# ssilverman16/particle_col_image_segmentation

Hardware: AMD Instinct MI355X
Metric: Mpixels/sec segmented (5-ch 1024x1024 TIFF), ROI mask IoU=1.0 (higher is better)
Workload: dtype f32 planes / u8 class maps / int32 labels / f64 ROI sums; 1 GPU; BASELINE config 2: batch of 64 frames 1024x1024x5 float32 per GPU, full kernel chain, inputs resident in HBM; frames_per_gpu=64, height=1024, width=1024, planes=5, parallelism=frames x1, launch=one hipGraph replay per step, 4 in flight, tie_fallback_frames_last_step=0, reference_nan_frames_rank0=0

## Files before the change

particle_col_image_segmentation_amd/csrc/ccl.hip:

```cpp
#include <type_traits>

#include "column_pass.h"
#include "tile_ops.h"

namespace pcseg {

constexpr int SCAN_PIX = 1024;

struct KeyEqU8 {
    const uint8_t *p;
    int W;
    int64_t n;
    __device__ __forceinline__ int operator()(int b, int r, int c) const { return p[b * n + rowoff(r, W) + c]; }
};
struct KeyNzU8 {
    const uint8_t *p;
    int W;
    int64_t n;
    __device__ __forceinline__ int operator()(int b, int r, int c) const { return p[b * n + rowoff(r, W) + c] != 0; }
};
struct KeyZeroU8 {
    const uint8_t *p;
    int W;
    int64_t n;
// ... 376 lines not shown
    const size_t words = (size_t)B * ((H + 31) / 32) * W;
    DilateCclWs ws;
    ws.bits = cv.take<unsigned>(words);
    ws.dil = cv.take<unsigned>(words);
    return ws;
}
static unsigned *dilate_ccl_runs_carve(Carver &cv, int B, int H, int W) { return cv.take<unsigned>((size_t)B * ((H + 31) / 32) * W); }

struct FillHolesWs : CclWs {
    uint8_t *flag;
};
static FillHolesWs fill_holes_carve(Carver &cv, int B, int H, int W)
{
    FillHolesWs ws;
    static_cast<CclWs &>(ws) = ccl_carve(cv, B, H, W);
    ws.flag = cv.take<uint8_t>((size_t)B * H * W);
    return ws;
}

struct LocmaxWs : CclWs {
    size_t nwords;
    unsigned long long *cbits;
    uint8_t *bad;
    int *nonconst;
};
static LocmaxWs locmax_carve(Carver &cv, int B, int H, int W)
{
    const size_t total = (size_t)B * H * W;
    LocmaxWs ws;
    static_cast<CclWs &>(ws) = ccl_carve(cv, B, H, W);
    ws.nwords = (total + 63) / 64;
    ws.cbits = cv.take<unsigned long long>(ws.nwords + 1);
    ws.bad = cv.take<uint8_t>(total);
    ws.nonconst = cv.take<int>(B);
    return ws;
}

struct OverlapWs : CclWs {
    int *area, *ov;
};
static OverlapWs overlap_carve(Carver &cv, int B, int H, int W)
{
    OverlapWs ws;
    static_cast<CclWs &>(ws) = ccl_carve(cv, B, H, W);
    ws.area = cv.take<int>((size_t)B * H * W);
    ws.ov = cv.take<int>((size_t)B * H * W);
    return ws;
}

template <typename KeyFn, bool CONN8>
static int ccl_roots(KeyFn keyfn, int *parent, int B, int H, int W, hipStream_t s, bool tile_pass_done = false, int *corrupt = nullptr)
{
    if (corrupt) PCSEG_CHECK_HIP(hipMemsetAsync(corrupt, 0, sizeof(int) * (size_t)B, s));
    dim3 tgrid((W + CCL_TW - 1) / CCL_TW, (H + CCL_TH - 1) / CCL_TH, B);
    if (!tile_pass_done) {
        PCSEG_LAUNCH((ccl_tile_kernel<KeyFn, CONN8>), tgrid, dim3(256), 0, s, keyfn, parent, H, W);
        PCSEG_CHECK_LAUNCH();
    }
    if (tgrid.x > 1 || tgrid.y > 1) {
        const int64_t border_px = (int64_t)((H - 1) / CCL_TH) * W + (int64_t)(CONN8 ? 2 : 1) * ((W - 1) / CCL_TW) * H;
        dim3 bgrid((unsigned)((border_px + 255) / 256), B);
        PCSEG_LAUNCH((ccl_border_kernel<KeyFn, CONN8>), bgrid, dim3(256), 0, s, keyfn, parent, H, W, corrupt);
        PCSEG_CHECK_LAUNCH();
    }
    return PCSEG_OK;
}

template <typename Pred>
static int ccl_compact(int *parent, int *blockcount, int nblk, int *labels, int *counts, Pred pred, bool flatten,
                       int B, int H, int W, hipStream_t s, int *corrupt = nullptr)
{
    int64_t n = (int64_t)H * W;
    dim3 grid(nblk, B);
    PCSEG_LAUNCH((ccl_flatten_count_kernel<Pred>), grid, dim3(256), 0, s, parent, labels, blockcount, pred, n, nblk, false, corrupt);
    PCSEG_CHECK_LAUNCH();
    PCSEG_LAUNCH(ccl_scan_blocks_kernel, dim3(B), dim3(256), 0, s, blockcount, counts, nblk, (const int *)corrupt);
    PCSEG_CHECK_LAUNCH();
    if ((n & 3) == 0 && (((uintptr_t)parent | (uintptr_t)labels) & 15) == 0) {
        const dim3 qgrid((unsigned)((n + SCAN_PIX * RELABEL_Q - 1) / (SCAN_PIX * RELABEL_Q)), B);
        PCSEG_LAUNCH((ccl_relabel_quads_kernel<Pred>), qgrid, dim3(256), 0, s, (const int *)parent, labels, (const int *)blockcount, pred, n,
                     nblk, flatten, counts);
    } else {
        PCSEG_LAUNCH((ccl_relabel_kernel<Pred>), grid, dim3(256), 0, s, (const int *)parent, labels, (const int *)blockcount, pred, n, nblk,
                     flatten, counts);
    }
    PCSEG_CHECK_LAUNCH();
    return PCSEG_OK;
}

template <typename KeyFn, bool CONN8>
static int ccl_full(KeyFn keyfn, int32_t *labels, int32_t *counts, int B, int H, int W, void *workspace,
                    size_t workspace_bytes, hipStream_t s)
{
    Carver cv(workspace, workspace_bytes);
    CclWs ws = ccl_carve(cv, B, H, W);
    if (!cv.ok()) {
        set_error("ccl: workspace too small (%zu < %zu)", workspace_bytes, cv.off);
        return PCSEG_ERR_WORKSPACE;
    }
    int rc = ccl_roots<KeyFn, CONN8>(keyfn, ws.parent, B, H, W, s, false, ws.corrupt);
    if (rc) return rc;
    return ccl_compact(ws.parent, ws.blockcount, ws.nblk, labels, counts, PredAll(), true, B, H, W, s, ws.corrupt);
}

int ccl_plan(void *workspace, size_t workspace_bytes, int B, int H, int W, CclPlan *plan, const char *who)
{
    Carver cv(workspace, workspace_bytes);
    CclWs ws = ccl_carve(cv, B, H, W);
    if (!cv.ok()) {
        set_error("%s: workspace too small (%zu < %zu)", who, workspace_bytes, cv.off);
        return PCSEG_ERR_WORKSPACE;
    }
    plan->parent = ws.parent;
    plan->blockcount = ws.blockcount;
    plan->nblk = ws.nblk;
    plan->corrupt = ws.corrupt;
    return PCSEG_OK;
}

int ccl_equal_u8_finish(const uint8_t *in, const CclPlan &plan, bool tile_pass_done, int *labels, int *counts, int B, int H, int W,
                        hipStream_t s)
{
    const KeyEqU8 keyfn{in, W, (int64_t)H * W};
    PCSEG_CHECK_HIP(hipMemsetAsync(plan.corrupt, 0, sizeof(int) * (size_t)B, s));
    dim3 tgrid((W + CCL_TW - 1) / CCL_TW, (H + CCL_TH - 1) / CCL_TH, B);
    if (!tile_pass_done) {
        PCSEG_LAUNCH((ccl_tile_kernel<KeyEqU8, true>), tgrid, dim3(256), 0, s, keyfn, plan.parent, H, W);
        PCSEG_CHECK_LAUNCH();
    }
    if (tgrid.x > 1 || tgrid.y > 1) {
        const int64_t border_px = (int64_t)((H - 1) / CCL_TH) * W + (int64_t)2 * ((W - 1) / CCL_TW) * H;
        dim3 bgrid((unsigned)((border_px + 255) / 256), B);
        PCSEG_LAUNCH((ccl_border_kernel<KeyEqU8, true>), bgrid, dim3(256), 0, s, keyfn, plan.parent, H, W, plan.corrupt);
        PCSEG_CHECK_LAUNCH();
    }
    return ccl_compact(plan.parent, plan.blockcount, plan.nblk, labels, counts, PredAll(), true, B, H, W, s, plan.corrupt);
}

__global__ void __launch_bounds__(256) roots_to_parent_kernel(const int *__restrict__ roots, int *__restrict__ parent, int64_t total)
{
    int64_t i = (int64_t)blockIdx.x * blockDim.x + threadIdx.x;
    if (i < total) parent[i] = roots[i] - 1;
}

struct MaskSet {
    unsigned long long bits[4];
    int n;
};
template <bool VEC>
__global__ void __launch_bounds__(256) set_bits_kernel(const uint8_t *__restrict__ in, MaskSet masks, unsigned *__restrict__ bits,
                                                        int H, int W, int nch, int B)
{
    constexpr int COLS = VEC ? 4 : 1;
    const int c = (blockIdx.x * 256 + threadIdx.x) * COLS;
    const int ch = blockIdx.y, b = blockIdx.z;
    if (c >= W) return;
    const uint8_t *src = in + (int64_t)b * H * W + c;
    unsigned w[4][COLS];
#pragma unroll
    for (int m = 0; m < 4; ++m)
#pragma unroll
        for (int j = 0; j < COLS; ++j) w[m][j] = 0;
#pragma unroll 1
    for (int j0 = 0; j0 < 32; j0 += 8) {
        unsigned v8[8];
#pragma unroll
        for (int j = 0; j < 8; ++j) {
            const uint8_t *at = src + rowoff(min(ch * 32 + j0 + j, H - 1), W);
            v8[j] = VEC ? *reinterpret_cast<const unsigned *>(at) : (unsigned)*at;
        }
#pragma unroll
        for (int j = 0; j < 8; ++j) {
#pragma unroll
            for (int q = 0; q < COLS; ++q) {
                const unsigned a = (v8[j] >> (8 * q)) & 255u;
                const unsigned long long sel = a < 64 ? (1ull << a) : 0ull;
#pragma unroll
                for (int m = 0; m < 4; ++m)
                    if (m < masks.n && (masks.bits[m] & sel)) w[m][q] |= 1u << (j0 + j);
            }
        }
    }
    {
        const int rows = min(32, H - ch * 32);
        const unsigned valid = col_valid(rows);
#pragma unroll
        for (int m = 0; m < 4; ++m)
#pragma unroll
            for (int q = 0; q < COLS; ++q) w[m][q] &= valid;
    }
    const int64_t plane = (int64_t)B * nch * W;
#pragma unroll
    for (int m = 0; m < 4; ++m)
        if (m < masks.n) {
            unsigned *out = bits + m * plane + ((int64_t)b * nch + ch) * W + c;
            if constexpr (VEC) *reinterpret_cast<uint4 *>(out) = make_uint4(w[m][0], w[m][1], w[m][2], w[m][3]);
            else *out = w[m][0];
        }
}

__global__ void __launch_bounds__(256) dilate_bits_kernel(const unsigned *__restrict__ in, unsigned *__restrict__ out,
                                                           int radius, int H, int W, int nch)
{
    const int c = blockIdx.x * 256 + threadIdx.x;
    const int ch = blockIdx.y, b = blockIdx.z;
    if (c >= W) return;
    const unsigned *base = in + (int64_t)b * nch * W;
    unsigned acc = 0;
    for (int dy = 0; dy <= radius; ++dy) {
        int half = 0;
        while ((half + 1) * (half + 1) + dy * dy <= radius * radius) ++half;
        unsigned cur = 0, prev = 0, next = 0;
        for (int dx = -half; dx <= half; ++dx) {
            int cc = c + dx;
            if (cc < 0 || cc >= W) continue;
            cur |= base[rowoff(ch, W) + cc];
            if (dy > 0) {
                if (ch > 0) prev |= base[rowoff((ch - 1), W) + cc];
                if (ch + 1 < nch) next |= base[rowoff((ch + 1), W) + cc];
            }
        }
        if (dy == 0) acc |= cur;
        else {
            acc |= (cur << dy) | (prev >> (32 - dy));
            acc |= (cur >> dy) | (next << (32 - dy));
        }
    }
    const int rows = min(32, H - ch * 32);
    acc &= col_valid(rows);
    out[((int64_t)b * nch + ch) * W + c] = acc;
}

__global__ void __launch_bounds__(256) dilate_bits_disk2_kernel(const unsigned *__restrict__ in, unsigned *__restrict__ out, int H, int W,
                                                                 int nch)
{
    const int c = blockIdx.x * 256 + threadIdx.x;
    const int ch = blockIdx.y, b = blockIdx.z;
    if (c >= W) return;
    const unsigned *base = in + (int64_t)b * nch * W;
    const int chu = max(ch - 1, 0), chd = min(ch + 1, nch - 1);
    const unsigned *rc = base + rowoff(ch, W), *ru = base + rowoff(chu, W), *rd = base + rowoff(chd, W);
    const int c1l = max(c - 1, 0), c2l = max(c - 2, 0), c1r = min(c + 1, W - 1), c2r = min(c + 2, W - 1);
    const unsigned w0 = rc[c], w1l = rc[c1l], w1r = rc[c1r], w2l = rc[c2l], w2r = rc[c2r];
    unsigned u0 = ru[c], u1l = ru[c1l], u1r = ru[c1r], d0 = rd[c], d1l = rd[c1l], d1r = rd[c1r];
    if (ch == 0) u0 = u1l = u1r = 0;
    if (ch + 1 >= nch) d0 = d1l = d1r = 0;
    const unsigned cur1 = w0 | w1l | w1r, prev1 = u0 | u1l | u1r, next1 = d0 | d1l | d1r;
    unsigned acc = cur1 | w2l | w2r;
    acc |= (cur1 << 1) | (prev1 >> 31) | (cur1 >> 1) | (next1 << 31);
    acc |= (w0 << 2) | (u0 >> 30) | (w0 >> 2) | (d0 << 30);
    const int rows = min(32, H - ch * 32);
    acc &= col_valid(rows);
    out[((int64_t)b * nch + ch) * W + c] = acc;
}

constexpr int BR_TW = 64, BR_CH = 4, BR_ROWS = 32 * BR_CH;

__device__ __forceinline__ int bitrun_start(unsigned word, int p)
{
    const unsigned below = ~word & ((1u << p) - 1u);
    return below ? 32 - __clz(below) : 0;
}

template <typename Link>
__device__ __forceinline__ void bitrun_left_links(unsigned w, unsigned wl, Link &&link)
{
    unsigned rest = wl ? w : 0u;
    while (rest) {
        const int a = __ffs(rest) - 1;
        const unsigned from_a = w >> a;
        const int len = from_a == 0xFFFFFFFFu ? 32 : __ffs(~from_a) - 1;
        const int e = a + len - 1;
        rest = e >= 31 ? 0u : rest & ~((2u << e) - 1u);
        const int lo = max(a - 1, 0), hi = min(e + 1, 31);
        unsigned m = wl & (hi == 31 ? 0xFFFFFFFFu : ((2u << hi) - 1u)) & ~((1u << lo) - 1u);
        while (m) {
            const int p = __ffs(m) - 1;
            const int st = bitrun_start(wl, p);
            const unsigned from_p = wl >> p;
            const int run_len = from_p == 0xFFFFFFFFu ? 32 : __ffs(~from_p) - 1;
            const int en = p + run_len - 1;
            m = en >= 31 ? 0u : m & ~((2u << en) - 1u);
            link(a, st);
        }
    }
}

__global__ void __launch_bounds__(256) bitrun_tile_kernel(const unsigned *__restrict__ bits, int *__restrict__ parent, int H, int W,
                                                           int nch)
{
    __shared__ unsigned sw[BR_CH][BR_TW];
    __shared__ int lpar[BR_ROWS * BR_TW];
    const int col = threadIdx.x & (BR_TW - 1), q = threadIdx.x >> 6;
    const int c0 = blockIdx.x * BR_TW, ch0 = blockIdx.y * BR_CH, b = blockIdx.z;
    const int c = c0 + col, ch = ch0 + q;
    const unsigned w = (c < W && ch < nch) ? bits[((int64_t)b * nch + ch) * W + c] : 0u;
    sw[q][col] = w;
    for (unsigned heads = w & ~(w << 1); heads; heads &= heads - 1) {
        const int node = (q * 32 + (__ffs(heads) - 1)) * BR_TW + col;
        lpar[node] = node;
    }
    __syncthreads();
    if (w) {
        if (col > 0)
            bitrun_left_links(w, sw[q][col - 1], [&](int a, int st) {
                unite_lds(lpar, (q * 32 + a) * BR_TW + col, (q * 32 + st) * BR_TW + col - 1);
            });
        if ((w & 1u) && q > 0) {
            const int node = (q * 32) * BR_TW + col;
            const unsigned wu = sw[q - 1][col];
            if (wu >> 31) {
                unite_lds(lpar, node, ((q - 1) * 32 + bitrun_start(wu, 31)) * BR_TW + col);
            } else {
                if (col > 0 && (sw[q - 1][col - 1] >> 31))
                    unite_lds(lpar, node, ((q - 1) * 32 + bitrun_start(sw[q - 1][col - 1], 31)) * BR_TW + col - 1);
                if (col + 1 < BR_TW && (sw[q - 1][col + 1] >> 31))
                    unite_lds(lpar, node, ((q - 1) * 32 + bitrun_start(sw[q - 1][col + 1], 31)) * BR_TW + col + 1);
            }
        }
    }
    __syncthreads();
    int *par = parent + (int64_t)b * H * W;
    for (unsigned heads = w & ~(w << 1); heads; heads &= heads - 1) {
        const int node = (q * 32 + (__ffs(heads) - 1)) * BR_TW + col;
        const int root = find_lds(lpar, node);
        par[(ch0 * 32 + node / BR_TW) * W + c0 + node % BR_TW] = (ch0 * 32 + root / BR_TW) * W + c0 + root % BR_TW;
    }
}

__global__ void __launch_bounds__(256) bitrun_border_kernel(const unsigned *__restrict__ bits, int *__restrict__ parent, int H, int W,
                                                             int nch)
{
    const int c = blockIdx.x * 256 + threadIdx.x;
    const int ch = blockIdx.y, b = blockIdx.z;
    if (c >= W) return;
    const int col = c & (BR_TW - 1);
    const bool tile_left = col == 0 && c > 0, tile_top = (ch % BR_CH) == 0 && ch > 0;
    const bool edge_col = col == 0 || col == BR_TW - 1;
    if (!tile_left && !tile_top && !(edge_col && ch > 0)) return;
    const unsigned *wb = bits + (int64_t)b * nch * W;
    const int cl = c > 0 ? c - 1 : c, cr = c + 1 < W ? c + 1 : c, chu = ch > 0 ? ch - 1 : ch;
    const unsigned w = wb[rowoff(ch, W) + c], wl = wb[rowoff(ch, W) + cl];
    const unsigned wu = wb[rowoff(chu, W) + c], wul = wb[rowoff(chu, W) + cl], wur = wb[rowoff(chu, W) + cr];
    if (w == 0) return;
    int *par = parent + (int64_t)b * H * W;
    const int row0 = ch * 32;
    if (tile_left)
        bitrun_left_links(w, wl, [&](int a, int st) { unite_glb(par, (row0 + a) * W + c, (row0 + st) * W + c - 1); });
    if ((w & 1u) && ch > 0) {
        const int node = row0 * W + c;
        if (wu >> 31) {
            if (tile_top) unite_glb(par, node, (row0 - 32 + bitrun_start(wu, 31)) * W + c);
        } else {
            if (c > 0 && (tile_top || col == 0) && (wul >> 31)) unite_glb(par, node, (row0 - 32 + bitrun_start(wul, 31)) * W + c - 1);
            if (c + 1 < W && (tile_top || col == BR_TW - 1) && (wur >> 31))
                unite_glb(par, node, (row0 - 32 + bitrun_start(wur, 31)) * W + c + 1);
        }
    }
}

__global__ void __launch_bounds__(256) border_flag_kernel(const int *__restrict__ parent, uint8_t *__restrict__ flag, int H, int W)
{
    int t = blockIdx.x * blockDim.x + threadIdx.x;
    int r, c;
    if (t < W) { r = 0; c = t; }
    else if (t < 2 * W) { r = H - 1; c = t - W; }
    else if (t < 2 * W + H) { r = t - 2 * W; c = 0; }
    else if (t < 2 * W + 2 * H) { r = t - 2 * W - H; c = W - 1; }
    else return;
    int64_t fbase = (int64_t)blockIdx.y * H * W;
    int p = parent[fbase + rowoff(r, W) + c];
    if (p >= 0) flag[fbase + p] = 1;
}

__global__ void __launch_bounds__(256) fill_holes_out_kernel(const uint8_t *__restrict__ mask, const int *__restrict__ parent,
                                                              const uint8_t *__restrict__ flag, uint8_t *__restrict__ out, int64_t n)
{
    int64_t i = (int64_t)blockIdx.x * blockDim.x + threadIdx.x;
    if (i >= n) return;
    int64_t fbase = (int64_t)blockIdx.y * n;
    int p = parent[fbase + i];
    out[fbase + i] = (mask[fbase + i] != 0) || (p >= 0 && flag[fbase + p] == 0);
}

__global__ void __launch_bounds__(256) ccl_flatten_kernel(int *__restrict__ parent, int64_t n)
{
    int64_t i = (int64_t)blockIdx.x * blockDim.x + threadIdx.x;
    if (i >= n) return;
    int *par = parent + (int64_t)blockIdx.y * n;
    int p = par[i];
    if (p < 0 || !walk_ok((int)i, p)) return;
    const int x = walk_root(par, p);
    if (x != p) par[i] = x;
}

constexpr int LM_TW = CCL_TW, LM_TH = CCL_TH, LM_SW = LM_TW + 4, LM_SH = LM_TH + 4, LM_CW = LM_TW + 2, LM_CH = LM_TH + 2;

__global__ void __launch_bounds__(256) locmax_candidates_kernel(const int *__restrict__ img, unsigned long long *__restrict__ cbits,
                                                                 uint8_t *__restrict__ bad, int *__restrict__ nonconst,
                                                                 int *__restrict__ parent, int *__restrict__ markers, int H, int W)
{
    __shared__ int tile[LM_SH * LM_SW];
    __shared__ uint8_t cand[LM_CH * LM_CW];
    __shared__ int key[CCL_TILE];
    static_assert(LM_SH * LM_SW >= CCL_TILE, "the parents reuse the value tile");
    int *par = tile;
    const int OUTSIDE = (int)0x80000000;
    const TileIndex ti = xcd_tile_index();
    const int r0 = ti.y * LM_TH, c0 = ti.x * LM_TW;
    const int64_t fbase = (int64_t)ti.z * H * W;
    if ((W & 3) == 0 && c0 + LM_TW <= W && (((uintptr_t)img) & 15) == 0) {
        constexpr int QUADS = LM_SH * (LM_TW / 4), TRIPS = (QUADS + 255) / 256;
        int4 tq[TRIPS];
#pragma unroll
        for (int t = 0; t < TRIPS; ++t) {
            const int i = min((int)threadIdx.x + 256 * t, QUADS - 1);
            const int r = r0 + i / (LM_TW / 4) - 2;
            tq[t] = *reinterpret_cast<const int4 *>(img + fbase + rowoff(min(max(r, 0), H - 1), W) + c0 + 4 * (i % (LM_TW / 4)));
        }
        const int hl = min((int)threadIdx.x, LM_SH * 4 - 1);
        const int hr = r0 + (hl >> 2) - 2, hx = (hl & 3) < 2 ? (hl & 3) - 2 : LM_TW + (hl & 3) - 2, hc = c0 + hx;
        const int hv = img[fbase + rowoff(min(max(hr, 0), H - 1), W) + min(max(hc, 0), W - 1)];
#pragma unroll
        for (int t = 0; t < TRIPS; ++t) {
            const int i = (int)threadIdx.x + 256 * t;
            if (i < QUADS) {
                const int lr = i / (LM_TW / 4), r = r0 + lr - 2;
                const bool in = r >= 0 && r < H;
                int *dst = tile + lr * LM_SW + 2 + 4 * (i % (LM_TW / 4));
                dst[0] = in ? tq[t].x : OUTSIDE; dst[1] = in ? tq[t].y : OUTSIDE; dst[2] = in ? tq[t].z : OUTSIDE; dst[3] = in ? tq[t].w : OUTSIDE;
            }
        }
        if (threadIdx.x < LM_SH * 4) tile[(hl >> 2) * LM_SW + hx + 2] = (hr >= 0 && hr < H && hc >= 0 && hc < W) ? hv : OUTSIDE;
    } else {
        constexpr int TRIPS = (LM_SH * LM_SW + 255) / 256;
        int tv[TRIPS];
#pragma unroll
        for (int t = 0; t < TRIPS; ++t) {
            const int i = min((int)threadIdx.x + 256 * t, LM_SH * LM_SW - 1);
            const int r = r0 + i / LM_SW - 2, c = c0 + i % LM_SW - 2;
            tv[t] = img[fbase + rowoff(min(max(r, 0), H - 1), W) + min(max(c, 0), W - 1)];
        }
#pragma unroll
        for (int t = 0; t < TRIPS; ++t) {
            const int i = (int)threadIdx.x + 256 * t;
            const int r = r0 + i / LM_SW - 2, c = c0 + i % LM_SW - 2;
            if (i < LM_SH * LM_SW) tile[i] = (r >= 0 && r < H && c >= 0 && c < W) ? tv[t] : OUTSIDE;
        }
    }
    __syncthreads();
    const int first_value = img[fbase];
    bool any_differs = false;
    for (int t = threadIdx.x; t < LM_CH * LM_CW; t += 256) {
        const int lr = t / LM_CW, lc = t % LM_CW;
        const int r = r0 + lr - 1, c = c0 + lc - 1;
        const int i = (lr + 1) * LM_SW + lc + 1;
        const int v = tile[i];
        uint8_t state = 2;
        if (r >= 0 && r < H && c >= 0 && c < W) {
            const int *up = tile + i - LM_SW, *dn = tile + i + LM_SW;
            const int m = max(max(max(up[-1], up[0]), max(up[1], tile[i - 1])), max(max(tile[i + 1], dn[-1]), max(dn[0], dn[1])));
            state = m < v ? 1 : (m == v ? 3 : 0);
            any_differs = any_differs || v != first_value;
        }
        cand[t] = state;
    }
    __syncthreads();
    unsigned links = 0;
#pragma unroll
    for (int kk = 0; kk < LM_TH * LM_TW / 256; ++kk) {
        const int t = threadIdx.x + 256 * kk;
        const int lr = t / LM_TW, lc = t % LM_TW;
        const int r = r0 + lr, c = c0 + lc;
        int k = 0;
        if (r < H && c < W) {
            const int i = (lr + 2) * LM_SW + lc + 2, j = (lr + 1) * LM_CW + lc + 1;
            const int v = tile[i];
            const uint8_t st = cand[j];
            const bool is_cand = (st & 1) != 0;
            bool touches = false;
            if (st == 3) {
#pragma unroll
                for (int dr = -1; dr <= 1; ++dr)
#pragma unroll
                    for (int dc = -1; dc <= 1; ++dc) {
                        if (dr == 0 && dc == 0) continue;
                        const bool eq = tile[i + dr * LM_SW + dc] == v;
                        const uint8_t sn = cand[j + dr * LM_CW + dc];
                        touches = touches || (eq && sn == 0);
                        if ((dr < 0 || (dr == 0 && dc < 0)) && eq && (sn & 1) && lr + dr >= 0 && lc + dc >= 0 && lc + dc < LM_TW)
                            links |= 1u << (4 * kk + (dr == 0 ? 0 : dc + 2));
                    }
// ... 64 lines not shown
    uint8_t v = 0;
    if (cand_bit(cbits, fbase + i)) v = bad[fbase + parent[fbase + i]] == 0 && nonconst[blockIdx.y] != 0;
    is_max[fbase + i] = v;
}

__device__ __forceinline__ unsigned long long cand_word(const unsigned long long *cbits, int b, int64_t i0, int64_t n)
{
    if (i0 >= n) return 0ull;
    const int64_t g0 = (int64_t)b * n + i0;
    const int sh = (int)(g0 & 63);
    unsigned long long w = cbits[g0 >> 6] >> sh;
    if (sh) w |= cbits[(g0 >> 6) + 1] << (64 - sh);
    if (n - i0 < 64) w &= (1ull << (n - i0)) - 1ull;
    return w;
}

static_assert(SCAN_PIX == 1024, "sixteen 64-bit words per count block");
template <typename Pred>
__global__ void __launch_bounds__(256) locmax_count_kernel(const int *__restrict__ parent, int *__restrict__ labels,
                                                            int *__restrict__ blockcount, const unsigned long long *__restrict__ cbits,
                                                            Pred pred, int64_t n, int nblk)
{
    const int b = blockIdx.y;
    const int *par = parent + (int64_t)b * n;
    const int64_t word = (int64_t)blockIdx.x * 256 + threadIdx.x;
    const int64_t i0 = word * 64;
    unsigned long long roots = 0;
    for (unsigned long long m = cand_word(cbits, b, i0, n); m; m &= m - 1) {
        const int j = __ffsll((long long)m) - 1;
        const int64_t i = i0 + j;
        if (par[i] == (int)i && pred((int64_t)b * n + i)) roots |= 1ull << j;
    }
    const int cnt = __popcll(roots);
    int inc = cnt;
    for (int off = 1; off < 16; off <<= 1) {
        const int t = __shfl_up(inc, off, 16);
        if ((threadIdx.x & 15) >= off) inc += t;
    }
    int rank = inc - cnt;
    for (unsigned long long m = roots; m; m &= m - 1) labels[(int64_t)b * n + i0 + (__ffsll((long long)m) - 1)] = -(++rank);
    if ((threadIdx.x & 15) == 15 && word / 16 < nblk) blockcount[b * nblk + (int)(word / 16)] = inc;
}

template <typename Pred>
__global__ void __launch_bounds__(256) locmax_relabel_kernel(const int *__restrict__ parent, int *labels, const int *__restrict__ blockoff,
                                                              const unsigned long long *__restrict__ cbits, Pred pred, int64_t n, int nblk)
{
    const int b = blockIdx.y;
    const int *par = parent + (int64_t)b * n;
    int *lab = labels + (int64_t)b * n;
    const int64_t i0 = ((int64_t)blockIdx.x * 256 + threadIdx.x) * 64;
    for (unsigned long long m = cand_word(cbits, b, i0, n); m; m &= m - 1) {
        const int64_t i = i0 + (__ffsll((long long)m) - 1);
        const int p = par[i];
        int v = 0;
        if (pred((int64_t)b * n + p)) {
            v = __hip_atomic_load(lab + p, __ATOMIC_RELAXED, __HIP_MEMORY_SCOPE_WORKGROUP);
            if (v < 0) v = blockoff[b * nblk + p / SCAN_PIX] - v;
        }
        lab[i] = v;
    }
}

__global__ void __launch_bounds__(256) overlap_count_kernel(const int *__restrict__ parent, const uint8_t *__restrict__ other,
                                                             int *__restrict__ area, int *__restrict__ ov, int64_t n)
{
    int64_t i = (int64_t)blockIdx.x * blockDim.x + threadIdx.x;
    if (i >= n) return;
    int64_t fbase = (int64_t)blockIdx.y * n;
    int p = parent[fbase + i];
    if (p < 0) return;
    atomicAdd(&area[fbase + p], 1);
    if (other[fbase + i] == 1) atomicAdd(&ov[fbase + p], 1);
}

__global__ void __launch_bounds__(256) overlap_out_kernel(const uint8_t *__restrict__ dapi, const int *__restrict__ parent,
                                                           const int *__restrict__ area, const int *__restrict__ ov,
                                                           double threshold, uint8_t *__restrict__ out, int64_t n)
{
    int64_t i = (int64_t)blockIdx.x * blockDim.x + threadIdx.x;
    if (i >= n) return;
    int64_t fbase = (int64_t)blockIdx.y * n;
    int p = parent[fbase + i];
    uint8_t v = dapi[fbase + i];
    if (p >= 0) {
        double frac = (double)ov[fbase + p] / (double)area[fbase + p];
        if (frac > threshold) v = 2;
    }
    out[fbase + i] = v;
}

}

using namespace pcseg;

extern "C" {

size_t pcseg_ccl_workspace_bytes(int B, int H, int W)
{
    if (!check_shape(B, H, W)) return 0;
    Carver cv(nullptr, 0);
    ccl_carve(cv, B, H, W);
    return cv.off;
}

int pcseg_ccl8_equal_u8(const uint8_t *in, int32_t *labels, int32_t *counts, int B, int H, int W, void *workspace,
                        size_t workspace_bytes, pcseg_stream_t stream)
{
    PCSEG_REQUIRE(in && labels && counts && workspace && check_shape(B, H, W), "bad arguments");
    return ccl_full<KeyEqU8, true>(KeyEqU8{in, W, (int64_t)H * W}, labels, counts, B, H, W, workspace, workspace_bytes, (hipStream_t)stream);
}

int pcseg_ccl8_bool(const uint8_t *in, int32_t *labels, int32_t *counts, int B, int H, int W, void *workspace,
                    size_t workspace_bytes, pcseg_stream_t stream)
{
    PCSEG_REQUIRE(in && labels && counts && workspace && check_shape(B, H, W), "bad arguments");
    return ccl_full<KeyNzU8, true>(KeyNzU8{in, W, (int64_t)H * W}, labels, counts, B, H, W, workspace, workspace_bytes, (hipStream_t)stream);
}

int pcseg_ccl4_bool(const uint8_t *in, int32_t *labels, int32_t *counts, int B, int H, int W, void *workspace,
                    size_t workspace_bytes, pcseg_stream_t stream)
{
    PCSEG_REQUIRE(in && labels && counts && workspace && check_shape(B, H, W), "bad arguments");
    return ccl_full<KeyNzU8, false>(KeyNzU8{in, W, (int64_t)H * W}, labels, counts, B, H, W, workspace, workspace_bytes, (hipStream_t)stream);
}

size_t pcseg_dilate_ccl_workspace_bytes(int B, int H, int W)
{
    if (!check_shape(B, H, W)) return 0;
    Carver cv(nullptr, 0);
    dilate_ccl_carve(cv, B, H, W);
    return cv.off;
}

static int dilated_bit_planes(const uint8_t *in, const MaskSet &masks, int radius, unsigned *bits, unsigned *dil, int B, int H, int W,
                              hipStream_t s)
{
    const int nch = (H + 31) / 32;
    if ((W & 3) == 0 && ((uintptr_t)in & 3) == 0 && ((uintptr_t)bits & 15) == 0)
        PCSEG_LAUNCH(set_bits_kernel<true>, dim3((W / 4 + 255) / 256, nch, B), dim3(256), 0, s, in, masks, bits, H, W, nch, B);
    else
        PCSEG_LAUNCH(set_bits_kernel<false>, dim3((W + 255) / 256, nch, B), dim3(256), 0, s, in, masks, bits, H, W, nch, B);
    PCSEG_CHECK_LAUNCH();
    const dim3 g((W + 255) / 256, nch, B * masks.n);
    if (radius == 2) PCSEG_LAUNCH(dilate_bits_disk2_kernel, g, dim3(256), 0, s, (const unsigned *)bits, dil, H, W, nch);
    else PCSEG_LAUNCH(dilate_bits_kernel, g, dim3(256), 0, s, (const unsigned *)bits, dil, radius, H, W, nch);
    PCSEG_CHECK_LAUNCH();
    return PCSEG_OK;
}

static int bitrun_components(const unsigned *dil, int *run_parent, int B, int H, int W, hipStream_t s)
{
    const int nch = (H + 31) / 32;
    PCSEG_LAUNCH(bitrun_tile_kernel, dim3((W + BR_TW - 1) / BR_TW, (nch + BR_CH - 1) / BR_CH, B), dim3(256), 0, s, dil, run_parent, H,
                 W, nch);
    PCSEG_CHECK_LAUNCH();
    PCSEG_LAUNCH(bitrun_border_kernel, dim3((W + 255) / 256, nch, B), dim3(256), 0, s, dil, run_parent, H, W, nch);
    PCSEG_CHECK_LAUNCH();
    return PCSEG_OK;
}

static MaskSet mask_set(const uint64_t *value_bits, int n_masks)
{
    MaskSet masks;
    masks.n = n_masks;
    for (int m = 0; m < 4; ++m) masks.bits[m] = m < n_masks ? (unsigned long long)value_bits[m] : 0ull;
    return masks;
}

int pcseg_dilate_ccl_roots_u8(const uint8_t *in, uint64_t value_bits, int radius, int32_t *roots, int B, int H, int W,
                              void *workspace, size_t workspace_bytes, pcseg_stream_t stream)
{
    PCSEG_REQUIRE(in && roots && workspace && radius >= 0 && radius <= 15 && check_shape(B, H, W), "bad arguments (radius <= 15)");
    hipStream_t s = (hipStream_t)stream;
    Carver cv(workspace, workspace_bytes);
    const DilateCclWs ws = dilate_ccl_carve(cv, B, H, W);
    if (!cv.ok()) {
        set_error("dilate_ccl_roots: workspace too small (%zu < %zu)", workspace_bytes, cv.off);
        return PCSEG_ERR_WORKSPACE;
    }
    const int rc = dilated_bit_planes(in, mask_set(&value_bits, 1), radius, ws.bits, ws.dil, B, H, W, s);
    if (rc) return rc;
    return ccl_roots<KeyBits, true>(KeyBits{ws.dil, W, (H + 31) / 32}, roots, B, H, W, s);
}

size_t pcseg_dilate_ccl_runs_workspace_bytes(int B, int H, int W)
{
    if (!check_shape(B, H, W)) return 0;
    Carver cv(nullptr, 0);
    dilate_ccl_runs_carve(cv, B, H, W);
    return cv.off;
}

int pcseg_dilate_ccl_runs_multi_u8(const uint8_t *in, const uint64_t *value_bits, int n_masks, int radius, uint32_t *dilated_bits,
                                   int32_t *run_parent, int B, int H, int W, void *workspace, size_t workspace_bytes,
                                   pcseg_stream_t stream)
{
    PCSEG_REQUIRE(in && value_bits && dilated_bits && run_parent && workspace && n_masks >= 1 && n_masks <= 4 && radius >= 0 &&
                      radius <= 15 && check_shape(B, H, W) && check_shape(B * n_masks, H, W),
                  "bad arguments (1..4 masks, radius <= 15)");
    hipStream_t s = (hipStream_t)stream;
    const int BM = B * n_masks;
    Carver cv(workspace, workspace_bytes);
    unsigned *bits = dilate_ccl_runs_carve(cv, BM, H, W);
    if (!cv.ok()) {
        set_error("dilate_ccl_runs: workspace too small (%zu < %zu)", workspace_bytes, cv.off);
        return PCSEG_ERR_WORKSPACE;
    }
    const int rc = dilated_bit_planes(in, mask_set(value_bits, n_masks), radius, bits, (unsigned *)dilated_bits, B, H, W, s);
    if (rc) return rc;
    return bitrun_components((const unsigned *)dilated_bits, (int *)run_parent, BM, H, W, s);
}

int pcseg_dilate_ccl_runs_u8(const uint8_t *in, uint64_t value_bits, int radius, uint32_t *dilated_bits, int32_t *run_parent,
                             int B, int H, int W, void *workspace, size_t workspace_bytes, pcseg_stream_t stream)
{
    return pcseg_dilate_ccl_runs_multi_u8(in, &value_bits, 1, radius, dilated_bits, run_parent, B, H, W, workspace, workspace_bytes,
                                          stream);
}

int pcseg_compact_labels(const int32_t *roots, int32_t *labels, int32_t *counts, int B, int H, int W, void *workspace,
                         size_t workspace_bytes, pcseg_stream_t stream)
{
    PCSEG_REQUIRE(roots && labels && counts && workspace && roots != labels && check_shape(B, H, W), "bad arguments");
    hipStream_t s = (hipStream_t)stream;
    Carver cv(workspace, workspace_bytes);
    CclWs ws = ccl_carve(cv, B, H, W);
    if (!cv.ok()) {
        set_error("compact_labels: workspace too small (%zu < %zu)", workspace_bytes, cv.off);
        return PCSEG_ERR_WORKSPACE;
    }
    int64_t total = (int64_t)B * H * W;
    PCSEG_CHECK_HIP(hipMemsetAsync(ws.corrupt, 0, sizeof(int) * (size_t)B, s));
    PCSEG_LAUNCH(roots_to_parent_kernel, dim3((unsigned)((total + 255) / 256)), dim3(256), 0, s, roots, ws.parent, total);
    PCSEG_CHECK_LAUNCH();
    return ccl_compact(ws.parent, ws.blockcount, ws.nblk, labels, counts, PredAll(), true, B, H, W, s, ws.corrupt);
}

size_t pcseg_fill_holes_workspace_bytes(int B, int H, int W)
{
    if (!check_shape(B, H, W)) return 0;
    Carver cv(nullptr, 0);
    fill_holes_carve(cv, B, H, W);
    return cv.off;
}

int pcseg_fill_holes(const uint8_t *mask, uint8_t *out, int B, int H, int W, void *workspace, size_t workspace_bytes,
                     pcseg_stream_t stream)
{
    PCSEG_REQUIRE(mask && out && workspace && check_shape(B, H, W), "bad arguments");
    hipStream_t s = (hipStream_t)stream;
    int64_t n = (int64_t)H * W;
    Carver cv(workspace, workspace_bytes);
    const FillHolesWs ws = fill_holes_carve(cv, B, H, W);
    uint8_t *flag = ws.flag;
    if (!cv.ok()) {
        set_error("fill_holes: workspace too small (%zu < %zu)", workspace_bytes, cv.off);
        return PCSEG_ERR_WORKSPACE;
    }
    int rc = ccl_roots<KeyZeroU8, false>(KeyZeroU8{mask, W, (int64_t)H * W}, ws.parent, B, H, W, s);
    if (rc) return rc;
    dim3 g1((unsigned)((n + 255) / 256), B);
    PCSEG_LAUNCH(ccl_flatten_kernel, g1, dim3(256), 0, s, ws.parent, n);
    PCSEG_CHECK_LAUNCH();
    PCSEG_CHECK_HIP(hipMemsetAsync(flag, 0, (size_t)B * n, s));
    PCSEG_LAUNCH(border_flag_kernel, dim3((2 * W + 2 * H + 255) / 256, B), dim3(256), 0, s, ws.parent, flag, H, W);
    PCSEG_CHECK_LAUNCH();
    PCSEG_LAUNCH(fill_holes_out_kernel, g1, dim3(256), 0, s, mask, ws.parent, flag, out, n);
    PCSEG_CHECK_LAUNCH();
    return PCSEG_OK;
}

size_t pcseg_local_maxima_workspace_bytes(int B, int H, int W)
{
    if (!check_shape(B, H, W)) return 0;
    Carver cv(nullptr, 0);
    locmax_carve(cv, B, H, W);
    return cv.off;
}

int pcseg_local_maxima_i32(const int32_t *img, uint8_t *is_max, int32_t *markers, int32_t *counts, int B, int H, int W,
                           void *workspace, size_t workspace_bytes, pcseg_stream_t stream)
{
    PCSEG_REQUIRE(img && workspace && check_shape(B, H, W), "bad arguments");
    PCSEG_REQUIRE(!markers || counts, "markers need counts");
    hipStream_t s = (hipStream_t)stream;
    int64_t n = (int64_t)H * W;
    const int64_t total = (int64_t)B * n;
    Carver cv(workspace, workspace_bytes);
    const LocmaxWs ws = locmax_carve(cv, B, H, W);
    const size_t nwords = ws.nwords;
    unsigned long long *cbits = ws.cbits;
    uint8_t *bad = ws.bad;
    int *nonconst = ws.nonconst;
    if (!cv.ok()) {
        set_error("local_maxima: workspace too small (%zu < %zu)", workspace_bytes, cv.off);
        return PCSEG_ERR_WORKSPACE;
    }
    PCSEG_CHECK_HIP(hipMemsetAsync(nonconst, 0, sizeof(int) * B, s));
    PCSEG_CHECK_HIP(hipMemsetAsync(cbits, 0, sizeof(unsigned long long) * (nwords + 1), s));
    dim3 g2((W + LM_TW - 1) / LM_TW, (H + LM_TH - 1) / LM_TH, B);
    PCSEG_LAUNCH(locmax_candidates_kernel, g2, dim3(256), 0, s, img, cbits, bad, nonconst, ws.parent, (int *)markers, H, W);
    PCSEG_CHECK_LAUNCH();
    int rc = ccl_roots<KeyCandBits, true>(KeyCandBits{img, cbits, W, n}, ws.parent, B, H, W, s, true);
    if (rc) return rc;
    const dim3 gw((unsigned)((nwords + 255) / 256));
    PCSEG_LAUNCH(locmax_propagate_kernel, gw, dim3(256), 0, s, ws.parent, bad, (const unsigned long long *)cbits, n, total);
    PCSEG_CHECK_LAUNCH();
    if (is_max) {
        dim3 g1((unsigned)((n + 255) / 256), B);
        PCSEG_LAUNCH(locmax_out_kernel, g1, dim3(256), 0, s, (const int *)ws.parent, (const uint8_t *)bad, (const int *)nonconst,
// ... 55 lines not shown
```

Before: 16540 Mpixels/s.

## Speed up bitrun merge: LUT set_bits, compact tile union-find, edge-only border launch

set_bits_kernel now builds a 256-entry shared lookup table that packs the four mask memberships of each byte value, so each column's eight rows are classified with table loads instead of per-mask 64-bit tests. bitrun_tile_kernel compacts its LDS parent array to half the rows by mapping only run heads through bitrun_slot, uses its own atomicMin union-find, and launches 64*BR_CH threads. bitrun_border_kernel's grid now covers only the tile-edge words (top rows of tiles plus edge columns) instead of every word and returning early. The cost is an extra __syncthreads and table fill per block, plus more index arithmetic for the edge enumeration. Profiling scripts are added alongside.

After: 17010 Mpixels/s (median of 6 runs). +2.8%, better.

```diff
diff --git a/particle_col_image_segmentation_amd/csrc/ccl.hip b/particle_col_image_segmentation_amd/csrc/ccl.hip
--- a/particle_col_image_segmentation_amd/csrc/ccl.hip
+++ b/particle_col_image_segmentation_amd/csrc/ccl.hip
@@ -552,6 +552,16 @@
                                                         int H, int W, int nch, int B)
 {
     constexpr int COLS = VEC ? 4 : 1;
+    __shared__ unsigned tbl[VEC ? 256 : 1];
+    if constexpr (VEC) {
+        const int a = threadIdx.x;
+        unsigned t = 0;
+#pragma unroll
+        for (int m = 0; m < 4; ++m)
+            if (m < masks.n && a < 64) t |= (unsigned)((masks.bits[m] >> a) & 1ull) << (8 * m);
+        tbl[a] = t;
+        __syncthreads();
+    }
     const int c = (blockIdx.x * 256 + threadIdx.x) * COLS;
     const int ch = blockIdx.y, b = blockIdx.z;
     if (c >= W) return;
@@ -569,15 +579,23 @@
             const uint8_t *at = src + rowoff(min(ch * 32 + j0 + j, H - 1), W);
             v8[j] = VEC ? *reinterpret_cast<const unsigned *>(at) : (unsigned)*at;
         }
-#pragma unroll
-        for (int j = 0; j < 8; ++j) {
+        if constexpr (VEC) {
 #pragma unroll
             for (int q = 0; q < COLS; ++q) {
-                const unsigned a = (v8[j] >> (8 * q)) & 255u;
+                unsigned rows8 = 0;
+#pragma unroll
+                for (int j = 0; j < 8; ++j) rows8 |= tbl[(v8[j] >> (8 * q)) & 255u] << j;
+#pragma unroll
+                for (int m = 0; m < 4; ++m) w[m][q] |= ((rows8 >> (8 * m)) & 255u) << j0;
+            }
+        } else {
+#pragma unroll
+            for (int j = 0; j < 8; ++j) {
+                const unsigned a = v8[j] & 255u;
                 const unsigned long long sel = a < 64 ? (1ull << a) : 0ull;
 #pragma unroll
                 for (int m = 0; m < 4; ++m)
-                    if (m < masks.n && (masks.bits[m] & sel)) w[m][q] |= 1u << (j0 + j);
+                    if (m < masks.n && (masks.bits[m] & sel)) w[m][0] |= 1u << (j0 + j);
             }
         }
     }
@@ -686,11 +704,33 @@
     }
 }
 
-__global__ void __launch_bounds__(256) bitrun_tile_kernel(const unsigned *__restrict__ bits, int *__restrict__ parent, int H, int W,
-                                                           int nch)
+constexpr int BR_NODES = BR_ROWS / 2 * BR_TW;
+__device__ __forceinline__ int bitrun_slot(int id) { return ((id >> 7) << 6) | (id & (BR_TW - 1)); }
+static_assert(BR_TW == 64 && BR_CH > 1, "bitrun_slot: a node id is row * 64 + column; BitrunEdges: tile rows of several word rows");
+__device__ __forceinline__ int bitrun_find(int *par, int x)
+{
+    int p;
+    while ((p = ld_lds(par + bitrun_slot(x))) != x) x = p;
+    return x;
+}
+__device__ __forceinline__ void bitrun_unite(int *par, int a, int b)
+{
+    for (;;) {
+        a = bitrun_find(par, a);
+        b = bitrun_find(par, b);
+        if (a == b) return;
+        if (a < b) { int t = a; a = b; b = t; }
+        const int old = atomicMin(&par[bitrun_slot(a)], b);
+        if (old == a) return;
+        a = old;
+    }
+}
+
+__global__ void __launch_bounds__(64 * BR_CH) bitrun_tile_kernel(const unsigned *__restrict__ bits, int *__restrict__ parent, int H,
+                                                                 int W, int nch)
 {
     __shared__ unsigned sw[BR_CH][BR_TW];
-    __shared__ int lpar[BR_ROWS * BR_TW];
+    __shared__ int lpar[BR_NODES];
     const int col = threadIdx.x & (BR_TW - 1), q = threadIdx.x >> 6;
     const int c0 = blockIdx.x * BR_TW, ch0 = blockIdx.y * BR_CH, b = blockIdx.z;
     const int c = c0 + col, ch = ch0 + q;
@@ -698,24 +738,24 @@
     sw[q][col] = w;
     for (unsigned heads = w & ~(w << 1); heads; heads &= heads - 1) {
         const int node = (q * 32 + (__ffs(heads) - 1)) * BR_TW + col;
-        lpar[node] = node;
+        lpar[bitrun_slot(node)] = node;
     }
     __syncthreads();
     if (w) {
         if (col > 0)
             bitrun_left_links(w, sw[q][col - 1], [&](int a, int st) {
-                unite_lds(lpar, (q * 32 + a) * BR_TW + col, (q * 32 + st) * BR_TW + col - 1);
+                bitrun_unite(lpar, (q * 32 + a) * BR_TW + col, (q * 32 + st) * BR_TW + col - 1);
             });
         if ((w & 1u) && q > 0) {
             const int node = (q * 32) * BR_TW + col;
             const unsigned wu = sw[q - 1][col];
             if (wu >> 31) {
-                unite_lds(lpar, node, ((q - 1) * 32 + bitrun_start(wu, 31)) * BR_TW + col);
+                bitrun_unite(lpar, node, ((q - 1) * 32 + bitrun_start(wu, 31)) * BR_TW + col);
             } else {
                 if (col > 0 && (sw[q - 1][col - 1] >> 31))
-                    unite_lds(lpar, node, ((q - 1) * 32 + bitrun_start(sw[q - 1][col - 1], 31)) * BR_TW + col - 1);
+                    bitrun_unite(lpar, node, ((q - 1) * 32 + bitrun_start(sw[q - 1][col - 1], 31)) * BR_TW + col - 1);
                 if (col + 1 < BR_TW && (sw[q - 1][col + 1] >> 31))
-                    unite_lds(lpar, node, ((q - 1) * 32 + bitrun_start(sw[q - 1][col + 1], 31)) * BR_TW + col + 1);
+                    bitrun_unite(lpar, node, ((q - 1) * 32 + bitrun_start(sw[q - 1][col + 1], 31)) * BR_TW + col + 1);
             }
         }
     }
@@ -723,21 +763,36 @@
     int *par = parent + (int64_t)b * H * W;
     for (unsigned heads = w & ~(w << 1); heads; heads &= heads - 1) {
         const int node = (q * 32 + (__ffs(heads) - 1)) * BR_TW + col;
-        const int root = find_lds(lpar, node);
+        const int root = bitrun_find(lpar, node);
         par[(ch0 * 32 + node / BR_TW) * W + c0 + node % BR_TW] = (ch0 * 32 + root / BR_TW) * W + c0 + root % BR_TW;
     }
 }
 
+struct BitrunEdges {
+    int n_top;
+    int n_cols;
+    __host__ __device__ BitrunEdges(int W, int nch) : n_top((nch - 1) / BR_CH), n_cols(2 * ((W - 1) / BR_TW) + (W % BR_TW == 0)) {}
+    __host__ __device__ int64_t count(int W, int nch) const { return (int64_t)n_top * W + (int64_t)(nch - n_top) * n_cols; }
+};
 __global__ void __launch_bounds__(256) bitrun_border_kernel(const unsigned *__restrict__ bits, int *__restrict__ parent, int H, int W,
                                                              int nch)
 {
-    const int c = blockIdx.x * 256 + threadIdx.x;
-    const int ch = blockIdx.y, b = blockIdx.z;
-    if (c >= W) return;
+    const BitrunEdges ed(W, nch);
+    const int i = blockIdx.x * 256 + threadIdx.x, b = blockIdx.y;
+    int c, ch;
+    if (i < ed.n_top * W) {
+        ch = (i / W + 1) * BR_CH;
+        c = i % W;
+    } else {
+        const int j = i - ed.n_top * W;
+        if (ed.n_cols == 0 || j >= (nch - ed.n_top) * ed.n_cols) return;
+        const int r = j / ed.n_cols, e = j % ed.n_cols;
+        ch = r == 0 ? 0 : r + (r - 1) / (BR_CH - 1);
+        c = BR_TW - 1 + BR_TW * (e >> 1) + (e & 1);
+    }
+    if (c >= W || ch >= nch) return;
     const int col = c & (BR_TW - 1);
     const bool tile_left = col == 0 && c > 0, tile_top = (ch % BR_CH) == 0 && ch > 0;
-    const bool edge_col = col == 0 || col == BR_TW - 1;
-    if (!tile_left && !tile_top && !(edge_col && ch > 0)) return;
     const unsigned *wb = bits + (int64_t)b * nch * W;
     const int cl = c > 0 ? c - 1 : c, cr = c + 1 < W ? c + 1 : c, chu = ch > 0 ? ch - 1 : ch;
     const unsigned w = wb[rowoff(ch, W) + c], wl = wb[rowoff(ch, W) + cl];
@@ -1108,11 +1163,14 @@
 static int bitrun_components(const unsigned *dil, int *run_parent, int B, int H, int W, hipStream_t s)
 {
     const int nch = (H + 31) / 32;
-    PCSEG_LAUNCH(bitrun_tile_kernel, dim3((W + BR_TW - 1) / BR_TW, (nch + BR_CH - 1) / BR_CH, B), dim3(256), 0, s, dil, run_parent, H,
-                 W, nch);
-    PCSEG_CHECK_LAUNCH();
-    PCSEG_LAUNCH(bitrun_border_kernel, dim3((W + 255) / 256, nch, B), dim3(256), 0, s, dil, run_parent, H, W, nch);
-    PCSEG_CHECK_LAUNCH();
+    PCSEG_LAUNCH(bitrun_tile_kernel, dim3((W + BR_TW - 1) / BR_TW, (nch + BR_CH - 1) / BR_CH, B), dim3(64 * BR_CH), 0, s, dil, run_parent,
+                 H, W, nch);
+    PCSEG_CHECK_LAUNCH();
+    const int64_t edge_words = BitrunEdges(W, nch).count(W, nch);
+    if (edge_words > 0) {
+        PCSEG_LAUNCH(bitrun_border_kernel, dim3((unsigned)((edge_words + 255) / 256), B), dim3(256), 0, s, dil, run_parent, H, W, nch);
+        PCSEG_CHECK_LAUNCH();
+    }
     return PCSEG_OK;
 }
 
diff --git a/profiles/merge_paths/summarise_kernels.py b/profiles/merge_paths/summarise_kernels.py
--- /dev/null
+++ b/profiles/merge_paths/summarise_kernels.py
@@ -0,0 +1,70 @@
+import glob
+import json
+import os
+import sys
+
+MERGE = ("set_bits_kernel<true>", "dilate_bits_disk2_kernel", "bitrun_tile_kernel", "bitrun_border_kernel", "merge_groups_kernel")
+
+
+def med(v):
+    v = sorted(v)
+    return (v[(len(v) - 1) // 2] + v[len(v) // 2]) / 2
+
+
+def load(d, pattern):
+    return [json.load(open(p)) for p in sorted(glob.glob(os.path.join(d, pattern)))]
+
+
+def main(d):
+    ok = True
+    par, bra = load(d, "kernels_parent_*.json"), load(d, "kernels_branch_*.json")
+    groups = {json.dumps(r.pop("groups"), sort_keys=True) for r in par + bra}
+    assert len(groups) == 1, "the libraries disagree on the group counts"
+    names = sorted(par[0], key=lambda k: -sum(par[0][k]))
+    runs = lambda rs, k: [x for r in rs for x in r[k]]
+    merge = [k for k in names if any(m in k for m in MERGE)]
+    print("## Serial per-kernel times, us per launch (`measure.sh kernels`: three processes a library, p b p b p b, three passes = runs each)\n")
+    print("| kernel | parent runs | branch runs | parent mean | branch mean | difference | parent spread |\n|---|---|---|---|---|---|---|")
+    rose = []
+    for k in merge + [k for k in names if k not in merge]:
+        a, b = runs(par, k), runs(bra, k)
+        diff, spread = sum(b) / len(b) - sum(a) / len(a), max(a) - min(a)
+        if k not in merge and diff > spread:
+            rose.append(k)
+        if k in merge or abs(diff) > spread:
+            print("| `%s` | %s | %s | %.1f | %.1f | %+.1f | %.1f |" % (k.split(" [")[0].strip("()"), ", ".join("%.1f" % x for x in a),
+                                                                  ", ".join("%.1f" % x for x in b), sum(a) / len(a), sum(b) / len(b), diff, spread))
+    sa = [sum(r[k][i] for k in merge) for r in par for i in range(len(r[merge[0]]))]
+    sb = [sum(r[k][i] for k in merge) for r in bra for i in range(len(r[merge[0]]))]
+    fall, spread = sum(sa) / len(sa) - sum(sb) / len(sb), max(sa) - min(sa)
+    print("\nThe five merge kernels together: parent %s, branch %s: **%.1f -> %.1f us (%.0f %%)**, parent spread %.1f us." % (
+        ", ".join("%.1f" % x for x in sa), ", ".join("%.1f" % x for x in sb), sum(sa) / len(sa), sum(sb) / len(sb), -100 * fall / (sum(sa) / len(sa)), spread))
+    print("Condition `fall > parent spread`: **%s**.  (Kernels outside the chain are listed only where they differ by more than" % ("holds" if fall > spread else "FAILS"))
+    print("their parent spread.)  Other kernels whose mean rose by more than their parent spread: %s.\n" % (", ".join("`%s`" % k for k in rose) or "none"))
+    ok = ok and fall > spread and not rose
+    tot = lambda rs: [sum(sum(v) / len(v) for v in r.values()) for r in rs]
+    print("Sum over every kernel of a step's launches' means (not the step time: kernels launch different numbers of times): parent %s, branch %s.\n" % (
+        ", ".join("%.0f" % x for x in tot(par)), ", ".join("%.0f" % x for x in tot(bra))))
+    hp = [r["ms_per_step"] for r in load(d, "headline_parent_*.json")]
+    hb = [r["ms_per_step"] for r in load(d, "headline_branch_*.json")]
+    if hp:
+        gain, spread = med(hp) - med(hb), max(hp) - min(hp)
+        print("## Headline: `bench.py --gpus 1 --steps 20 --warmup 4`, ms per step (`measure.sh headline`: p b p b p b p b)\n")
+        print("| | runs | median |\n|---|---|---|")
+        print("| parent | %s | %.4g |\n| branch | %s | %.4g |" % (", ".join("%.4g" % x for x in hp), med(hp), ", ".join("%.4g" % x for x in hb), med(hb)))
+        good = gain > spread
+        print("\nBranch median below the parent's by %.3f ms (%.1f %%); the parent's max - min is %.3f ms: the headline gain is **%s**." % (
+            gain, 100 * gain / med(hp), spread, "outside the parent's spread" if good else "INSIDE the parent's spread -- not claimed"))
+        print("Run by run (branch - the parent run before it): %s.\n" % ", ".join("%+.3f" % (y - x) for x, y in zip(hp, hb)))
+        up, uc = (json.load(open(os.path.join(d, "unfused_%s.json" % k))) for k in ("parent", "child"))
+        assert up["groups"] == uc["groups"]
+        print("## Entry points off the benchmark path (time_unfused.py: 2 frames of 160 x 160, median of 50, us; no condition)\n")
+        print("| call | parent | branch |\n|---|---|---|")
+        for k in uc:
+            if k.endswith("_us"):
+                print("| `%s` | %.1f | %.1f |" % (k[:-3], up[k], uc[k]))
+    return 0 if ok else 1
+
+
+if __name__ == "__main__":
+    sys.exit(main(sys.argv[1]))
diff --git a/profiles/merge_paths/time_kernels.py b/profiles/merge_paths/time_kernels.py
--- /dev/null
+++ b/profiles/merge_paths/time_kernels.py
@@ -0,0 +1,33 @@
+import ctypes
+import json
+import os
+import sys
+
+import torch
+
+sys.path.insert(0, os.path.join(os.path.dirname(os.path.abspath(__file__)), "..", ".."))
+from particle_col_image_segmentation_amd import _lib, synth
+from particle_col_image_segmentation_amd.pipeline import FramePipeline
+
+PASSES = int(sys.argv[1]) if len(sys.argv) > 1 else 3
+lib = _lib.load()
+stack = synth.gen_batch_torch(10000, 64, 1024, 1024, torch.device("cuda:0"))
+solo = FramePipeline(dict(synth.CELL_TYPES_5), overlap=False)
+for _ in range(2):
+    res = solo.run(stack)
+torch.cuda.synchronize()
+out = {}
+for _ in range(PASSES):
+    lib.pcseg_timing_enable(1)
+    for _ in range(2):
+        res = solo.run(stack)
+    torch.cuda.synchronize()
+    nbytes = lib.pcseg_timing_report(None, 0)
+    buf = ctypes.create_string_buffer(nbytes + 16)
+    lib.pcseg_timing_report(buf, nbytes + 16)
+    lib.pcseg_timing_enable(0)
+    for line in buf.value.decode().splitlines():
+        name, calls, ms = line.split("\t")
+        out.setdefault(name, []).append(round(1e3 * float(ms) / int(calls), 2))
+out["groups"] = {str(k): int(v["n_groups"].sum()) for k, v in res["groups"].items()}
+print(json.dumps(out))
```
